# cropinghigh/sdrpp-dvbs-demodulator

Measured on AMD Instinct MI355X. Metric: Msymbols/s demod+FEC, DVB-S2 8PSK 3/4 normal-frame @50 LDPC iters, higher is better.
Workload: dtype int8 (FEC) / f32 (demod); 1 GPU; DVB-S2 8PSK 3/4 normal FECFRAME (MODCOD 14), pilots off, 27.5 Msym/s-class streams at 2 sps, carrier offset 1e-3 rad/sample, clock error ~10 ppm, Es/N0 11 dB, 50 forced LDPC iterations, IQ in -> BBFRAMEs out; streams_per_gpu=4096, symbols_per_frame=21690, distinct_signal_blocks=64, parallelism=independent transponder streams sharded over GPUs, no data-path collective, fec_pipelined_across_steps=True, ranks_seen_by_backend=1, backend=none

## Files before the change

### sdrpp-dvbs-demodulator_amd/csrc/ldpc_split_kernel.hip

```cpp
#include <hip/hip_runtime.h>
#include <stdint.h>
#include <algorithm>
#include "ldpc_lane_common.h"
#include "ldpc_split_plan.h"

namespace s2 {

#ifndef LDPC_SPLIT_EXP
#define LDPC_SPLIT_EXP 0
#endif
#ifndef LDPC_SPLIT_SKIP
#define LDPC_SPLIT_SKIP 0
#endif

template <int MAXDEG>
struct SplitShape {
    static constexpr int NL = MAXDEG + 2, HS = (NL + 1) / 2, NP = (HS + 1) / 2;
    static constexpr bool ODD = (NL & 1) != 0;
    static constexpr int PREV_SLOT = ODD ? HS - 2 : HS - 1;
    static constexpr int NPW = (HS / 2 + 1) <= 1 ? 1 : (HS / 2 + 1) <= 2 ? 2 : (HS / 2 + 1) <= 4 ? 4 : 8;
    static constexpr int REC = HS <= 4 ? 1 : HS <= 8 ? 2 : 4;
    static constexpr int RI_WORD = HS / 2, RI_SHIFT = (HS & 1) ? 16 : 0;
    static constexpr int NOPREV_SHARED = (MAXDEG == 4 || MAXDEG == 8) ? 2 : 0;
    static_assert(HS / 2 + 1 <= NPW, "slots + row word must fit the thread's table entry (ldpc_split_plan.h)");
// ... 103 lines not shown
        }
        if (S::ODD && ((HS - 1) >> 1) == p) {
            const bool me = (t & 1) != 0;
            constexpr int hh = (HS - 1) & 1;
            v[hh] = me ? (short)(127 << 8) : v[hh];
            g[hh] = me ? (short)(126 << 8) : g[hh];
        }
        R.V[p] = v; R.G[p] = g;
        if constexpr (LATE < 0) {
            if (p < -LATE) { v = late ? splat2(127 << 8) : v; g = late ? splat2(126 << 8) : g; }
        }
        if (p == 0) { MIN0 = g; }
        else if (p == 1) { MIN1 = pmax2(MIN0, g); MIN0 = pmin2(MIN0, g); }
        else { MIN1 = pmin2(MIN1, pmax2(MIN0, g)); MIN0 = pmin2(MIN0, g); }
        SX ^= bits2(v);
    }
    const int m0 = (int)bits2(pmin2(MIN0, swap2(MIN0)));
    const int m1 = (int)bits2(pmin2(pmax2(MIN0, swap2(MIN0)), pmin2(MIN1, swap2(MIN1))));
    const int sx = (int)(SX ^ __builtin_amdgcn_alignbit(SX, SX, 16));
    const int o0 = QUAD_DPP(m0, DPP_SWAP_HALVES), o1 = QUAD_DPP(m1, DPP_SWAP_HALVES), os = QUAD_DPP(sx, DPP_SWAP_HALVES);
    M1 = min(max(m0, o0), min(m1, o1));
    M0 = min(m0, o0);
    SXs = sx ^ os;
}

template <int MAXDEG, int LATE>
__device__ __forceinline__ void row_totals(const RowState<MAXDEG>& R, const uint32_t late, int& M0, int& M1, int& SXs) {
    using S = SplitShape<MAXDEG>;
    constexpr int NP = S::NP;
    s16x2 MIN0 = splat2(Q8_NONE), MIN1 = splat2(Q8_NONE);
    uint32_t SX = 0;
#pragma unroll
    for (int p = 0; p < NP; ++p) {
        s16x2 v = R.V[p], g = R.G[p];
        if constexpr (LATE < 0) {
            if (p < -LATE) { v = late ? splat2(127 << 8) : v; g = late ? splat2(126 << 8) : g; }
        }
        if (p == 0) { MIN0 = g; }
        else if (p == 1) { MIN1 = pmax2(MIN0, g); MIN0 = pmin2(MIN0, g); }
        else { MIN1 = pmin2(MIN1, pmax2(MIN0, g)); MIN0 = pmin2(MIN0, g); }
        SX ^= bits2(v);
    }
    const int m0 = (int)bits2(pmin2(MIN0, swap2(MIN0)));
    const int m1 = (int)bits2(pmin2(pmax2(MIN0, swap2(MIN0)), pmin2(MIN1, swap2(MIN1))));
    const int sx = (int)(SX ^ __builtin_amdgcn_alignbit(SX, SX, 16));
    const int o0 = QUAD_DPP(m0, DPP_SWAP_HALVES), o1 = QUAD_DPP(m1, DPP_SWAP_HALVES), os = QUAD_DPP(sx, DPP_SWAP_HALVES);
    M1 = min(max(m0, o0), min(m1, o1));
    M0 = min(m0, o0);
    SXs = sx ^ os;
}

template <int MAXDEG, int SKIP>
__device__ __forceinline__ void row_output(const RowState<MAXDEG>& R, const int M0, const int M1, const int SXs, const uint32_t early, uint32_t (&rec_out)[SplitShape<MAXDEG>::REC],
                                           uint32_t* pn0 = nullptr , const int npn = 1) {
    using S = SplitShape<MAXDEG>;
    constexpr int HS = S::HS, NP = S::NP, REC = S::REC;
    const uint32_t C32 = 0x20002000u;
    const uint32_t MIN1C = (uint32_t)min(M1, (int)C32);
    const uint32_t SUMC = (uint32_t)min(M0, (int)C32) + MIN1C;
    const uint32_t SXB = (uint32_t)SXs;
    s16x2 NM[NP + 1];
    NM[NP] = splat2(0);
#pragma unroll
    for (int p = 0; p < NP; ++p) {
        const s16x2 other = from_bits2(SUMC - bits2(pmin2(R.G[p], from_bits2(MIN1C))));
        const s16x2 neg = from_bits2(SXB ^ bits2(R.V[p])) >> 15;
        s16x2 nm = pmin2(from_bits2(bits2(other) ^ bits2(neg)) - neg, q8(31));
        const uint32_t pn = bits2(sat_add2(R.V[p], nm)) >> 8;
        if (p < npn && pn0) pn0[p] = pn;
#pragma unroll
        for (int hh = 0; hh < 2; ++hh) {
            const int k = 2 * p + hh;
            if (k >= HS) { nm[hh] = 0; continue; }
            if (k < SKIP) {
                if (!((early >> k) & 1)) { if (hh == 0) lds_write_lo_i8(R.addr[k], pn); else lds_write_hi_i8(R.addr[k], pn); }
            } else {
                if (hh == 0) lds_write_lo_i8(R.addr[k], pn); else lds_write_hi_i8(R.addr[k], pn);
            }
        }
        NM[p] = nm;
    }
#pragma unroll
    for (int w = 0; w < REC; ++w) {
        if (2 * w < NP) rec_out[w] = __builtin_amdgcn_perm(bits2(NM[2 * w + 1 <= NP ? 2 * w + 1 : NP]), bits2(NM[2 * w]), 0x07050301u);
        else rec_out[w] = 0;
    }
}

#if defined(LDPC_PROF) && LDPC_PROF == 3
#define SPLIT_MARK(i) do { if (KIND == 1 && g_prof_dev && blockIdx.x == 0 && (t == 0 || t == 384)) { const unsigned long long t_now = clock64(); g_prof_dev[300 + (t ? 16 : 0) + (i)] += t_now - t_mark; t_mark = t_now; } } while (0)
#define SPLIT_MARK_DECL unsigned long long t_mark = clock64()
__device__ unsigned long long* g_prof_dev = nullptr;
#else
#define SPLIT_MARK(i) do { } while (0)
#define SPLIT_MARK_DECL do { } while (0)
#endif
#define LINK_IN(k) ((int)R.V[(k) >> 1][(k) & 1] >> 8)
#define LINK_MG(k) ((int)R.G[(k) >> 1][(k) & 1] >> 8)
#define LINK_SET(k, v, m) do { R.V[(k) >> 1][(k) & 1] = (short)((v) << 8); R.G[(k) >> 1][(k) & 1] = (short)((m) << 8); } while (0)

__device__ __forceinline__ uint2 chain_record_x(const int m, const int qE, const int vE, const int sneg ) {
    const int sig = 1 | sneg;
    const int c31 = min(qE, 31), c32 = min(qE, 32);
    const int CA = (sneg ? c32 : c31) + 1, CB = (sneg ? c31 : c32) + 1;
    const uint32_t lim = ((uint32_t)(m + 1) & 0xffu) | (((uint32_t)(m + CA) & 0xffu) << 8) | (((uint32_t)(m - CB) & 0xffu) << 16) | ((uint32_t)(m - 1) << 24);
    const uint32_t se = ((uint32_t)(vE - 2 * sig * m - sneg) & 0xffffu) | (((uint32_t)sneg & 0xffu) << 16);
    return make_uint2(lim, se);
}
__device__ __forceinline__ int chain_step_x(const int x, const u32x2 r) {
    const int q1 = min(max(x, (int)(int8_t)r.x), (int)(int8_t)(r.x >> 8));
    const int q2 = min(max(x, (int)(int8_t)(r.x >> 16)), (int)r.x >> 24);
    int tx = (q1 + q2) ^ (int)(int8_t)(r.y >> 16);
    asm volatile("" : "+v"(tx));
    return clamp8(tx + (int)(short)r.y);
}
typedef __attribute__((address_space(3))) u32x2 lds_u2;
#define LDS_U2(a) (*(const lds_u2*)(uintptr_t)(a))
typedef u32x2 __attribute__((aligned(4))) u32x2_a4;
typedef __attribute__((address_space(3))) u32x2_a4 lds_u2_a4;
#define LDS_U2_A4(a) (*(const lds_u2_a4*)(uintptr_t)(a))

template <int MAXDEG>
__device__ __forceinline__ void chain_layer(RowState<MAXDEG>& R, uint32_t (&rec_out)[SplitShape<MAXDEG>::REC],
                                            const LdpcSplitLayer L, const uint32_t eL, const int t, int8_t* __restrict__ post, uint32_t* __restrict__ cw,
                                            const uint32_t flagb , const uint32_t cseq ,
                                            const bool fail_attempts ) {
    [[maybe_unused]] constexpr int KIND = 1;
    typedef __attribute__((address_space(3))) uint32_t lds_u1;
    const uint32_t rw = R.rw;
    const uint32_t level = rw & 0xffu, late = (rw >> 8) & 3u, early = (rw >> 12) & 3u;
    const int chain_d = (int)(L.aux & 0xffffu);
    const int j = t >> 1;
    const bool half1 = (t & 1) != 0;
    const uint32_t emask = ((early & 1u) ? 0xffu : 0u) | ((early & 2u) ? 0xff0000u : 0u);
    const uint32_t my_flag = flagb + 4u * (cseq & 1u);
    const bool attempt = (uint32_t)__builtin_amdgcn_readfirstlane((int)*(const lds_u1*)(uintptr_t)(flagb + 4u * ((cseq - 1u) & 1u))) != cseq - 1u;
    int M0, M1, SXs;
    uint32_t x0, pn0 = 0;
    SPLIT_MARK_DECL;
    row_input<MAXDEG, -1, SplitShape<MAXDEG>::NOPREV_SHARED>(R, (!attempt && level > 1u && !half1) ? 1u : 0u, 1u , t, M0, M1, SXs, ((L.kind_nw >> 20) & 1u) != 0, &x0);
    SPLIT_MARK(0);
    if (attempt) {
        row_output<MAXDEG, 2>(R, M0, M1, SXs, (level > 1u && !half1) ? 3u : 0u, rec_out, &pn0);
        const bool bad = fail_attempts || ((pn0 ^ (x0 >> 8)) & emask) != 0;
        if (__builtin_amdgcn_ballot_w64(bad) != 0 && (t & 63) == 0) *(lds_u1*)(uintptr_t)my_flag = cseq;
        lds_pairs_wait();
        lds_barrier();
        if ((uint32_t)__builtin_amdgcn_readfirstlane((int)*(const lds_u1*)(uintptr_t)my_flag) != cseq) {
            if (level > 1u && !half1) {
                if (!(early & 1u)) lds_write_lo_i8(R.addr[0], pn0);
                if (!(early & 2u)) lds_write_hi_i8(R.addr[1], pn0);
            }
            return;
        }
        row_totals<MAXDEG, -1>(R, (level > 1u && !half1) ? 1u : 0u, M0, M1, SXs);
    } else if (level == 1u) {
        row_output<MAXDEG, 0>(R, M0, M1, SXs, 0u, rec_out, &pn0);
    }
    if ((late >> 1) & 1) {
        reinterpret_cast<uint2*>(cw)[j] = chain_record_x(R.msg(1), (late & 1u) ? 255 : (M0 >> 24), (int)R.V[0][0] >> 8, SXs >> 31);
    }
    SPLIT_MARK(1);
    lds_pairs_wait();
    lds_barrier();
    SPLIT_MARK(2);
    uint32_t cwb = lds_offset(reinterpret_cast<const int8_t*>(cw));
    asm volatile("" : "+s"(cwb));
    if (t < chain_d) {
        __builtin_amdgcn_s_setprio(3);
        const int T = (int)(L.aux >> 16);
        int x = post[link_addr(eL, t + chain_d)];
        const uint32_t step = 8u * (uint32_t)chain_d, step4 = 4u * step;
        uint32_t p0 = cwb + 8u * (uint32_t)(t + chain_d), p1 = p0 + step, p2 = p1 + step, p3 = p2 + step;
        u32x2 r0 = LDS_U2(p0), r1 = LDS_U2(p1), r2 = LDS_U2(p2), r3 = LDS_U2(p3);
        int k = 1;
#define WALK_ROW(p, r) do { LDS_I8((p) + 7u) = (int8_t)x; x = chain_step_x(x, r); asm volatile("" : "+v"(p), "+v"(x) : : "memory"); } while (0)
        for (; k + 4 <= T; k += 4) {
            WALK_ROW(p0, r0); p0 += step4; r0 = LDS_U2(p0);
            WALK_ROW(p1, r1); p1 += step4; r1 = LDS_U2(p1);
            WALK_ROW(p2, r2); p2 += step4; r2 = LDS_U2(p2);
            WALK_ROW(p3, r3); p3 += step4; r3 = LDS_U2(p3);
        }
        if (k < T) {
            WALK_ROW(p0, r0); ++k;
            if (k < T) {
                WALK_ROW(p1, r1); ++k;
                if (k < T) { WALK_ROW(p2, r2); ++k; }
            }
        }
#undef WALK_ROW
        if (t + T * chain_d < 360) LDS_I8(cwb + 8u * (uint32_t)(t + T * chain_d) + 7u) = (int8_t)x;
        __builtin_amdgcn_s_setprio(0);
    }
    SPLIT_MARK(3);
    lds_barrier();
    SPLIT_MARK(4);
    if (level > 1u) {
        if (!half1) {
            uint32_t xr, xh;
            lds_read_pair_i8(R.addr[0], cwb + 8u * (uint32_t)j + 7u, xr, xh);
            lds_ready_n(0, xr, xh);
            const s16x2 X = from_bits2(__builtin_amdgcn_perm(xh, xr, 0x060c000cu));
            const s16x2 v = sat_sub2(X, R.RP[0]);
            const s16x2 av = pmax2(v, sat_sub2(splat2(0), v));
            const s16x2 g = __builtin_bit_cast(s16x2, __builtin_elementwise_sub_sat(__builtin_bit_cast(u16x2, av), (u16x2){256, 256}));
            const uint32_t rws = rw << 22;
            const uint32_t LM = __builtin_amdgcn_perm(rws << 1, rws, 0x09090b0bu);
            R.V[0] = from_bits2((bits2(v) & LM) | (bits2(R.V[0]) & ~LM));
            R.G[0] = from_bits2((bits2(g) & LM) | (bits2(R.G[0]) & ~LM));
            const int a = (int)bits2(pmin2(R.G[0], swap2(R.G[0]))), b = (int)bits2(pmax2(R.G[0], swap2(R.G[0])));
            M1 = min(M1, max(M0, a));
            M0 = min(M0, a);
            M1 = min(M1, max(M0, b));
            const uint32_t sv = bits2(R.V[0]);
            SXs ^= (int)(sv ^ __builtin_amdgcn_alignbit(sv, sv, 16));
        }
        M0 = QUAD_DPP(M0, DPP_FROM_HALF0);
        M1 = QUAD_DPP(M1, DPP_FROM_HALF0);
        SXs = QUAD_DPP(SXs, DPP_FROM_HALF0);
        SPLIT_MARK(5);
        row_output<MAXDEG, 2>(R, M0, M1, SXs, early, rec_out, &pn0);
    }
    if (!attempt) {
        const bool bad = ((pn0 ^ (x0 >> 8)) & emask) != 0;
        if (__builtin_amdgcn_ballot_w64(bad) != 0 && (t & 63) == 0) *(lds_u1*)(uintptr_t)my_flag = cseq;
    }
    SPLIT_MARK(6);
}

typedef const __attribute__((address_space(4))) uint32_t* const_u32_ptr;
typedef const __attribute__((address_space(4))) LdpcSplitLayer* const_layer_ptr;

__device__ __forceinline__ LdpcSplitLayer layer_at(const_layer_ptr layers, int i) {
    LdpcSplitLayer L;
    L.kind_nw = layers[i].kind_nw; L.aux = layers[i].aux; L.rec_off = layers[i].rec_off; L.ent_off = layers[i].ent_off;
    return L;
}
#ifndef LDPC_SPLIT_SPEC_STATS
#define LDPC_SPLIT_SPEC_STATS 0
#endif
template <int MAXDEG>
__device__ __forceinline__ void spec_layer(RowState<MAXDEG>& R, uint32_t (&rec_out)[SplitShape<MAXDEG>::REC], const LdpcSplitLayer L, const uint32_t* __restrict__ tab, const int t,
                                           uint32_t* __restrict__ cw, [[maybe_unused]] unsigned long long* prof, [[maybe_unused]] const int pl,
                                           const uint32_t vflagb , const uint32_t cseq ,
                                           const bool fail_attempts ) {
    static_assert(SplitShape<MAXDEG>::HS >= 4, "the shared links are slots 0..3 of half 0");
    typedef __attribute__((address_space(3))) uint32_t lds_u1;
    const uint32_t level = R.rw & 0xffu;
    const int j = t >> 1;
    const bool half1 = (t & 1) != 0;
    const bool spec = level > 1u && !half1;
    const int depth = (int)(L.aux >> 16);
    u32x2 side;
    {
        const uint64_t sbase = (uint64_t)(uintptr_t)(tab + L.ent_off);
        const uint32_t voff = (uint32_t)j * 8u;
        asm volatile("global_load_dwordx2 %0, %1, %2" : "=&v"(side) : "v"(voff), "s"(sbase) : "memory");
    }
    uint32_t cwb = lds_offset(reinterpret_cast<const int8_t*>(cw));
    asm volatile("" : "+s"(cwb));
    const uint32_t flagb = cwb + 4u * 384u;
    if (t == 0) { *(lds_u1*)(uintptr_t)flagb = 0u; *(lds_u1*)(uintptr_t)(flagb + 4u) = 0u; }
    const uint32_t my_flag = vflagb + 4u * (cseq & 1u);
    const bool attempt = (uint32_t)__builtin_amdgcn_readfirstlane((int)*(const lds_u1*)(uintptr_t)(vflagb + 4u * ((cseq - 1u) & 1u))) != cseq - 1u;
    u32x2 side_a = {0u, 0u};
    if (attempt) {
        const uint64_t sbase = (uint64_t)(uintptr_t)(tab + L.ent_off);
        const uint32_t voff = (uint32_t)j * 8u;
        asm volatile("global_load_dwordx2 %0, %1, %2" : "=&v"(side_a) : "v"(voff), "s"(sbase) : "memory");
    }
    int M0, M1, SXs;
    uint32_t xr[2], pn[2] = {0u, 0u};
    row_input<MAXDEG, -2, SplitShape<MAXDEG>::NOPREV_SHARED>(R, (!attempt && spec) ? 1u : 0u, 1u, t, M0, M1, SXs, ((L.kind_nw >> 20) & 1u) != 0, xr, 2);
    uint32_t em0 = 0, em1 = 0;
#if LDPC_SPLIT_SPEC_STATS
    if (prof && blockIdx.x == 0 && t == 0) { prof[900] += 1; prof[901] += attempt; prof[910 + (cseq < 40 ? cseq : 40)] += attempt; }
#endif
    if (attempt) {
        row_output<MAXDEG, 4>(R, M0, M1, SXs, spec ? 15u : 0u, rec_out, pn, 2);
        asm volatile("s_waitcnt vmcnt(0)" : "+v"(side_a) : : "memory");
        em0 = (((side_a.x >> 15) & 1u) ? 0xffu : 0u) | (((side_a.x >> 31) & 1u) ? 0xff0000u : 0u);
        em1 = (((side_a.y >> 15) & 1u) ? 0xffu : 0u) | (((side_a.y >> 31) & 1u) ? 0xff0000u : 0u);
        const bool bad = fail_attempts || (!half1 && ((((pn[0] ^ (xr[0] >> 8)) & em0) | ((pn[1] ^ (xr[1] >> 8)) & em1)) != 0));
        if (__builtin_amdgcn_ballot_w64(bad) != 0 && (t & 63) == 0) *(lds_u1*)(uintptr_t)my_flag = cseq;
        lds_pairs_wait();
        lds_barrier();
        if ((uint32_t)__builtin_amdgcn_readfirstlane((int)*(const lds_u1*)(uintptr_t)my_flag) != cseq) {
#if LDPC_SPLIT_SPEC_STATS
            if (prof && blockIdx.x == 0 && t == 0) prof[902] += 1;
#endif
            if (spec) {
                if (!(em0 & 0xffu)) lds_write_lo_i8(R.addr[0], pn[0]);
                if (!(em0 >> 16)) lds_write_hi_i8(R.addr[1], pn[0]);
                if (!(em1 & 0xffu)) lds_write_lo_i8(R.addr[2], pn[1]);
                if (!(em1 >> 16)) lds_write_hi_i8(R.addr[3], pn[1]);
            }
            return;
        }
        row_totals<MAXDEG, -2>(R, spec ? 1u : 0u, M0, M1, SXs);
    } else {
        if (level == 1u) row_output<MAXDEG, 0>(R, M0, M1, SXs, 0u, rec_out, pn, 2);
    }
    const uint32_t cell = cwb + 4u * (uint32_t)j;
    uint32_t cur[4];
#pragma unroll
    for (int s = 0; s < 4; ++s) cur[s] = R.addr[s];
    const s16x2 Q0 = from_bits2((uint32_t)min(M0 >> 24, 32) * 0x01000100u);
    const uint32_t s0w = (uint32_t)(SXs >> 31) & 0x80008000u;
    lds_pairs_wait();
    lds_barrier();
    s16x2 V0 = R.V[0], V1 = R.V[1];
    uint32_t X0p = 0, X1p = 0;
    int p = 0;
    bool voted = false;
    const bool any_spec = __builtin_amdgcn_ballot_w64(spec) != 0;
    for (;;) {
        bool ch = false;
        if (any_spec) {
            if (spec) {
                uint32_t xr0, xh0, xr1, xh1;
                lds_read_pair_i8(cur[0], cur[1], xr0, xh0);
                lds_read_pair_i8(cur[2], cur[3], xr1, xh1);
                lds_ready_n(0, xr0, xh0);
                asm volatile("" : "+v"(xr1), "+v"(xh1));
                const uint32_t X0 = __builtin_amdgcn_perm(xh0, xr0, 0x060c000cu), X1 = __builtin_amdgcn_perm(xh1, xr1, 0x060c000cu);
                ch = ((X0 ^ X0p) | (X1 ^ X1p)) != 0;
                X0p = X0; X1p = X1;
                V0 = sat_sub2(from_bits2(X0), R.RP[0]);
                V1 = sat_sub2(from_bits2(X1), R.RP[1]);
                const s16x2 G0 = __builtin_bit_cast(s16x2, __builtin_elementwise_sub_sat(__builtin_bit_cast(u16x2, pmax2(V0, sat_sub2(splat2(0), V0))), (u16x2){256, 256}));
                const s16x2 G1 = __builtin_bit_cast(s16x2, __builtin_elementwise_sub_sat(__builtin_bit_cast(u16x2, pmax2(V1, sat_sub2(splat2(0), V1))), (u16x2){256, 256}));
                const s16x2 P0 = pmin2(G0, swap2(G0)), P1 = pmin2(G1, swap2(G1));
                const s16x2 O0 = pmin2(pmin2(swap2(G0), P1), Q0), O1 = pmin2(pmin2(swap2(G1), P0), Q0);
                uint32_t sx = bits2(V0) ^ bits2(V1);
                sx ^= __builtin_amdgcn_alignbit(sx, sx, 16);
                sx ^= s0w;
                const s16x2 N0 = from_bits2(sx ^ bits2(V0)) >> 15, N1 = from_bits2(sx ^ bits2(V1)) >> 15;
                const s16x2 NM0 = pmin2(from_bits2(bits2(O0) ^ bits2(N0)) - N0, q8(31)), NM1 = pmin2(from_bits2(bits2(O1) ^ bits2(N1)) - N1, q8(31));
                *(lds_u1*)(uintptr_t)cell = __builtin_amdgcn_perm(bits2(sat_add2(V1, NM1)), bits2(sat_add2(V0, NM0)), 0x07050301u);
            }
        }
        if (p == 0) {
            asm volatile("s_waitcnt vmcnt(0)" : "+v"(side) : : "memory");
#pragma unroll
            for (int s = 0; s < 4; ++s) {
                const uint32_t f = ((s < 2 ? side.x : side.y) >> (16 * (s & 1))) & 0x7ffu;
                cur[s] = f ? cell - f : R.addr[s];
            }
        }
        ++p;
        if (p >= depth - 1) break;
        if (p > 1 && __builtin_amdgcn_ballot_w64(ch) != 0 && (t & 63) == 0) *(lds_u1*)(uintptr_t)(flagb + 4u * (uint32_t)(p & 1)) = (uint32_t)p + 1u;
        lds_pairs_wait();
        lds_barrier();
        if (p > 1) {
            const uint32_t fl = (uint32_t)__builtin_amdgcn_readfirstlane((int)*(const lds_u1*)(uintptr_t)(flagb + 4u * (uint32_t)(p & 1)));
            if (fl != (uint32_t)p + 1u) { voted = true; break; }
        }
    }
#if LDPC_SPLIT_SPEC_STATS
    if (prof && blockIdx.x == 0 && t == 0) prof[512 + 32 * (pl % 11) + (p < 31 ? p : 31)] += 1;
#endif
    if (!voted) { lds_pairs_wait(); lds_barrier(); }
    if (level > 1u) {
        if (!half1) {
            R.V[0] = V0; R.V[1] = V1;
#pragma unroll
            for (int q = 0; q < 2; ++q) {
                R.G[q] = __builtin_bit_cast(s16x2, __builtin_elementwise_sub_sat(__builtin_bit_cast(u16x2, pmax2(R.V[q], sat_sub2(splat2(0), R.V[q]))), (u16x2){256, 256}));
                const int a = (int)bits2(pmin2(R.G[q], swap2(R.G[q]))), b = (int)bits2(pmax2(R.G[q], swap2(R.G[q])));
                M1 = min(M1, max(M0, a));
                M0 = min(M0, a);
                M1 = min(M1, max(M0, b));
            }
            const uint32_t sv = bits2(R.V[0]) ^ bits2(R.V[1]);
            SXs ^= (int)(sv ^ __builtin_amdgcn_alignbit(sv, sv, 16));
        }
        M0 = QUAD_DPP(M0, DPP_FROM_HALF0);
        M1 = QUAD_DPP(M1, DPP_FROM_HALF0);
        SXs = QUAD_DPP(SXs, DPP_FROM_HALF0);
        const uint32_t early = ((side.x >> 15) & 1u) | ((side.x >> 30) & 2u) | ((side.y >> 13) & 4u) | ((side.y >> 28) & 8u);
        row_output<MAXDEG, 4>(R, M0, M1, SXs, half1 ? 0u : early, rec_out, pn, 2);
    }
    if (!attempt) {
        em0 = (((side.x >> 15) & 1u) ? 0xffu : 0u) | (((side.x >> 31) & 1u) ? 0xff0000u : 0u);
        em1 = (((side.y >> 15) & 1u) ? 0xffu : 0u) | (((side.y >> 31) & 1u) ? 0xff0000u : 0u);
        const bool bad = !half1 && ((((pn[0] ^ (xr[0] >> 8)) & em0) | ((pn[1] ^ (xr[1] >> 8)) & em1)) != 0);
        if (__builtin_amdgcn_ballot_w64(bad) != 0 && (t & 63) == 0) *(lds_u1*)(uintptr_t)my_flag = cseq;
    }
}
#undef LINK_IN
#undef LINK_MG
#undef LINK_SET

template <int MAXDEG>
__global__ __launch_bounds__(LDPC_SPLIT_T) __attribute__((amdgpu_waves_per_eu(8))) void ldpc_split_kernel(LdpcKernelParams read_through_ldpc_params) {
    using S = SplitShape<MAXDEG>;
    constexpr int T = LDPC_SPLIT_T, REC = S::REC, NPW = S::NPW;
    extern __shared__ __attribute__((aligned(16))) int8_t lds_all[];
    const int t = threadIdx.x;
    const int wave = __builtin_amdgcn_readfirstlane(t >> 6);
    int8_t* __restrict__ post = lds_all;

#if defined(LDPC_PROF) && LDPC_PROF == 3
    if (blockIdx.x == 0) g_prof_dev = ldpc_params()->A.prof;
    __syncthreads();
#endif
    int f = blockIdx.x;
    while (f < ldpc_params()->A.nframes) {
        {
            const LdpcKernelParamsPtr P = ldpc_params();
            const int N = P->A.N, K = P->A.K, R = P->A.R, q = P->A.q;
            uint32_t* __restrict__ msg = P->A.msg_ws + (size_t)blockIdx.x * (size_t)P->A.pent_base;
            const int8_t* __restrict__ src = P->A.llr + (size_t)f * N;
            int t = threadIdx.x;
            asm volatile("" : "+v"(t));
            ldpc_frame_load<T>(post, src, K, R, q, t);
            for (uint32_t o = (uint32_t)t; o < (uint32_t)P->A.pent_base; o += T) msg[o] = 0;
            if (t < 2) reinterpret_cast<uint32_t*>(lds_all + ((N + LDPC_SPLIT_SCRATCH + 15) & ~15) + 8 * 360)[t] = 0;
        }
        __syncthreads();

        int it = 0, ret = 0;
        uint32_t cseq = 0;
        while (true) {
            const LdpcKernelParamsPtr P = ldpc_params();
            const LdpcKernelArgs A = ldpc_args(P);
            const int N = A.N, q = A.q, npl = P->npl;
            const const_layer_ptr layers = (const_layer_ptr)P->layers;
            const const_u32_ptr ents = (const_u32_ptr)P->ents;
            const int npad = (N + LDPC_SPLIT_SCRATCH + 15) & ~15;
            uint32_t* __restrict__ cw = reinterpret_cast<uint32_t*>(lds_all + npad);
            int* __restrict__ s_flag = reinterpret_cast<int*>(lds_all + N);
            const uint32_t cflagb = (uint32_t)npad + 8u * 360u;
            uint32_t* __restrict__ msg = A.msg_ws + (size_t)blockIdx.x * (size_t)A.pent_base;
            uint32_t* __restrict__ sgn = A.sgn_ws + (size_t)blockIdx.x * SGN_WS_DWORDS;
            const __amdgpu_buffer_rsrc_t rs_tab = wave_entries_rsrc<NPW>(const_cast<uint32_t*>(P->atab), wave, P->tab_words);
            const __amdgpu_buffer_rsrc_t rs_msg = wave_entries_rsrc<REC>(msg, wave, A.pent_base);
            const bool check = !A.force || it == A.max_trials;
            if (check) {
// ... 1 lines not shown
                const unsigned long long tc0 = clock64();
#endif
                const uint32_t zflag = sign_pack(post, N, reinterpret_cast<uint8_t*>(sgn), t, T);
#if defined(LDPC_PROF) && LDPC_PROF == 5
                const unsigned long long tc1 = clock64();
#endif
                __syncthreads();
#if defined(LDPC_PROF) && LDPC_PROF == 5
                const unsigned long long tc2 = clock64();
#endif
                const bool bad = zflag != 0 || syndromes_bad<MAXDEG>(q, A.synd_base, P->ents, sgn, t, T);
                const unsigned long long b = __ballot(bad);
#if defined(LDPC_PROF) && LDPC_PROF == 5
                const unsigned long long tc3 = clock64();
#endif
                if ((t & 63) == 0) s_flag[t >> 6] = (b != 0);
                lds_barrier();
                int any = 0;
#pragma unroll
                for (int w = 0; w < T / 64; ++w) any |= s_flag[w];
                any = __builtin_amdgcn_readfirstlane(any);
                lds_barrier();
#if defined(LDPC_PROF) && LDPC_PROF == 5
                if (A.prof && blockIdx.x == 0 && t == 0) { const unsigned long long tc4 = clock64(); A.prof[400] += tc1 - tc0; A.prof[401] += tc2 - tc1; A.prof[402] += tc3 - tc2; A.prof[403] += tc4 - tc3; A.prof[404] += 1; }
#endif
                if (A.force) { ret = any ? -1 : A.max_trials; break; }
                if (!any) { ret = it; break; }
                if (it == A.max_trials) { ret = -1; break; }
            }
            typename FetchWords<REC>::type rec_n;
            typename FetchWords<NPW>::type pw_n;
            LdpcSplitLayer Lnext = layer_at(layers, 0), Lnext2 = layer_at(layers, npl > 1 ? 1 : 0);
            uint32_t soff_tab = 0;
            pw_n = bload<NPW>(rs_tab, soff_tab);
            rec_n = bload<REC>(rs_msg, Lnext.rec_off * 4u);
            asm volatile("" : "+v"(rec_n), "+v"(pw_n));
#if defined(LDPC_PROF)
            unsigned long long t_layer = clock64();
            if (A.prof && blockIdx.x == 0 && t == 0) { A.prof[127] += t_layer - A.prof[126]; }
#endif
            for (int pl = 0; pl < npl; ++pl) {
                const LdpcSplitLayer L = Lnext;
                Lnext = Lnext2;
                Lnext2 = layer_at(layers, pl + 2 < npl ? pl + 2 : npl - 1);
                soff_tab += T * NPW * 4;
                RowState<MAXDEG> RS;
                RS.unpack(pw_n, rec_n);
                RS.pin();
                asm volatile("" : "+v"(pw_n), "+v"(rec_n));
                if (pl + 1 < npl && !(LDPC_SPLIT_EXP & 2)) {
                    if (!(LDPC_SPLIT_EXP & 16)) pw_n = bload<NPW>(rs_tab, soff_tab);
                    if (!(LDPC_SPLIT_EXP & 32)) rec_n = bload<REC>(rs_msg, Lnext.rec_off * 4u);
                }
                auto thread_index = [&]() __attribute__((always_inline)) { int tt = t; asm volatile("" : "+v"(tt)); return tt; };
                const uint32_t kind = L.kind_nw & 0xffu;
                uint32_t ro[REC];
                if (LDPC_SPLIT_SKIP && ((LDPC_SPLIT_SKIP >> kind) & 1)) {
#pragma unroll
                    for (int w = 0; w < REC; ++w) ro[w] = RS.rw;
                } else if (kind == 0) {
                    int M0, M1, SXs;
                    row_input<MAXDEG, 0>(RS, 0u, 0u, S::ODD ? thread_index() : t, M0, M1, SXs);
                    if (LDPC_SPLIT_EXP & 8) { ro[0] = (uint32_t)(M0 ^ M1 ^ SXs); ro[REC - 1] = ro[0]; }
                    else row_output<MAXDEG, 0>(RS, M0, M1, SXs, 0u, ro);
                } else if (kind == 7) {
                    int M0, M1, SXs;
                    row_input<MAXDEG, 0, 1>(RS, 0u, L.aux, thread_index(), M0, M1, SXs);
                    row_output<MAXDEG, 0>(RS, M0, M1, SXs, 0u, ro);
                } else if (kind == 1) {
                    ++cseq;
                    chain_layer<MAXDEG>(RS, ro, L, ents[L.ent_off + 1], thread_index(), post, cw, cflagb, cseq, A.dbg != 0);
                } else {
                    ++cseq;
                    if constexpr (S::HS >= 4) spec_layer<MAXDEG>(RS, ro, L, P->atab, thread_index(), cw, A.prof, pl, cflagb, cseq, A.dbg != 0);
                }
#if defined(LDPC_PROF) && LDPC_PROF == 4
                const unsigned long long t_claim = clock64();
#endif
                asm volatile("" : "+v"(rec_n), "+v"(pw_n));
#if defined(LDPC_PROF) && LDPC_PROF == 4
                if (A.prof && blockIdx.x == 0 && (t == 0 || t == 384)) A.prof[200 + pl + (t ? 50 : 0)] += clock64() - t_claim;
#endif
                if (LDPC_SPLIT_EXP & (2 | 64)) asm volatile("" :: "v"(ro[0]), "v"(ro[REC - 1]));
                else bstore<REC>(ro, rs_msg, L.rec_off * 4u);
                lds_pairs_wait();
                if (!(LDPC_SPLIT_EXP & 4)) lds_barrier();
#if defined(LDPC_PROF)
                if (A.prof && blockIdx.x == 0 && t == 0) { const unsigned long long t_now = clock64(); A.prof[128 + pl] += t_now - t_layer; t_layer = t_now; A.prof[126] = t_now; }
#endif
            }
            ++it;
        }

        {
            const LdpcKernelParamsPtr P = ldpc_params();
            const LdpcKernelArgs A = ldpc_args(P);
            const int N = A.N, K = A.K, R = A.R, q = A.q;
            int* __restrict__ s_flag = reinterpret_cast<int*>(lds_all + N);
            int t = threadIdx.x;
            asm volatile("" : "+v"(t));
            ldpc_frame_store<T>(post, f, ret, A.trials, A.hard, A.hard_stride, A.post, N, K, R, q, t, wave);
            if (A.work_ctr) {
                if (t == 0) s_flag[12] = (int)(gridDim.x + atomicAdd(A.work_ctr, 1u));
                lds_barrier();
                f = __builtin_amdgcn_readfirstlane(s_flag[12]);
            } else {
                f += gridDim.x;
            }
        }
        __syncthreads();
    }
}

size_t ldpc_split_lds_bytes(int N) {
    const size_t npad = (size_t)((N + LDPC_SPLIT_SCRATCH + 15) & ~15);
    return npad + 8 * 360 + 16;
}
size_t ldpc_split_msg_bytes_per_block(const LdpcDeviceCode& C) { return (size_t)C.split_rec_total * sizeof(uint32_t); }

template <int MAXDEG>
static hipError_t launch_split(const LdpcDeviceCode& C, const LdpcKernelArgs& A, int grid, hipStream_t stream) {
    LdpcKernelParams P;
    P.A = A; P.layers = C.d_split_layers; P.ents = C.d_ents; P.atab = C.d_split_atab; P.rows = C.d_rows; P.npl = C.split_npl; P.tab_words = C.split_tab_words;
    return ldpc_launch(ldpc_split_kernel<MAXDEG>, grid, LDPC_SPLIT_T, ldpc_split_lds_bytes(A.N), stream, P);
}
template <int MAXDEG>
static int occupancy_split(int N) { return ldpc_occupancy(ldpc_split_kernel<MAXDEG>, LDPC_SPLIT_T, ldpc_split_lds_bytes(N)); }
// ... 31 lines not shown
```

### sdrpp-dvbs-demodulator_amd/csrc/ldpc_split_plan.h

```cpp
#pragma once
#include "ldpc_plan.h"

namespace s2 {

constexpr int LDPC_SPLIT_T = 768;
constexpr int LDPC_SPLIT_SCRATCH = 64;
#ifndef LDPC_SPLIT_SPEC_MIN_T
#define LDPC_SPLIT_SPEC_MIN_T 64
#endif

struct LdpcSplitLayer {
    uint32_t kind_nw;
    uint32_t aux;
    uint32_t rec_off;
    uint32_t ent_off;
};

struct LdpcSplitPlan {
    bool ok = false;
    const char* why = "";
    int hs = 0;
    int npw = 0;
    int rec_dwords = 0;
    int rec_total = 0;
    int chain_layers = 0;
    bool noprev_shared = false;
    std::vector<LdpcSplitLayer> layers;
    std::vector<uint32_t> atab;
    std::vector<uint32_t> side;
    std::vector<int> row_of;
    std::vector<int> layer_of;
};

inline int ldpc_split_npw(int hs) {
    const int words = hs / 2 + 1;
    return words <= 1 ? 1 : words <= 2 ? 2 : words <= 4 ? 4 : 8;
}

inline int ldpc_split_plan_rec_dwords(int max_deg) { const int hs = (max_deg + 3) / 2; return hs <= 4 ? 1 : hs <= 8 ? 2 : 4; }

inline LdpcSplitPlan build_ldpc_split_plan(const LdpcPlan& P) {
    LdpcSplitPlan S;
    const int NL = P.max_deg + 2;
    if (P.min_deg != P.max_deg || (NL + 1) / 2 > 14 || P.N + LDPC_SPLIT_SCRATCH > 65536) { S.why = "irregular row degree, more than 14 slots per half or more than 65 472 bits"; return S; }
    for (const LdpcLayerDesc& L : P.layers) {
        const int nc = (int)(L.depth_nc >> 16), depth = (int)(L.depth_nc & 0xffffu);
        if (depth > 1 && (nc > 4 || nc > (NL + 1) / 2)) { S.why = "a layer with more than four shared links"; return S; }
    }
    S.hs = (NL + 1) / 2;
    S.npw = ldpc_split_npw(S.hs);
    S.rec_dwords = ldpc_split_plan_rec_dwords(P.max_deg);
    const int q = P.q, K = P.K, N = P.N, T = LDPC_SPLIT_T, hs = S.hs, npw = S.npw;
    auto scratch = [&](int t) { return (uint32_t)(N + (t & (LDPC_SPLIT_SCRATCH - 1))); };
    auto slot_addr = [&](int i, int j, int k) -> uint32_t {
        const LdpcLayerDesc& L = P.layers[i];
        if (k < P.max_deg) {
            const uint32_t e = P.ents[L.ent_off + k];
            return 360u * (e >> 16) + ((uint32_t)j + (e & 0xffffu)) % 360u;
        }
        if (k == P.max_deg) return (uint32_t)(K + 360 * i + j);
        if (i > 0) return (uint32_t)(K + 360 * (i - 1) + j);
        if (j > 0) return (uint32_t)(K + 360 * (q - 1) + j - 1);
        return ~0u;
    };
    std::vector<std::pair<int, std::vector<uint32_t>>> side_of;
    bool bad_noprev = false;
    auto emit = [&](int kind, int i, const std::vector<int>& rows, const std::vector<uint32_t>* info, uint32_t aux) {
        LdpcSplitLayer D{};
        const int nw = T / 64;
        D.kind_nw = (uint32_t)kind | ((uint32_t)nw << 8) | ((kind != 0 ? (P.layers[i].depth_nc >> 16) : 0u) << 16);
        D.aux = aux;
        D.rec_off = (uint32_t)S.rec_total;
        D.ent_off = P.layers[i].ent_off;
        S.rec_total += nw * 64 * S.rec_dwords;
        const size_t base = S.atab.size();
        S.atab.resize(base + (size_t)T * npw, 0);
        const size_t rbase = S.row_of.size();
        S.row_of.resize(rbase + T / 2, -1);
        for (int t = 0; t < T; ++t) {
            uint32_t* w = &S.atab[base + (size_t)t * npw];
            const int pr = t >> 1, h = t & 1;
            const int j = pr < (int)rows.size() ? rows[pr] : -1;
            for (int s = 0; s < hs; ++s) {
                uint32_t a = scratch(t);
                if (j >= 0 && h * hs + s < NL) {
                    a = slot_addr(i, j, h * hs + s);
                    if (a == ~0u) { a = scratch(t); D.kind_nw |= 1u << 20; if (kind == 0) { D.aux = (uint32_t)t; D.kind_nw = (D.kind_nw & ~0xffu) | 7u; } else bad_noprev = true; }
                }
                w[s >> 1] |= a << (16 * (s & 1));
            }
            if (j >= 0 && h == 0) S.row_of[rbase + pr] = j;
            if (j >= 0 && info && (h == 0 || kind == 1 || kind == 8)) w[hs >> 1] |= ((*info)[pr] & (h == 1 ? 0xffu : 0xffffu)) << (16 * (hs & 1));
        }
        S.layers.push_back(D);
        S.layer_of.push_back(i);
    };
    for (int i = 0; i < q; ++i) {
        const LdpcLayerDesc& L = P.layers[i];
        const int depth = (int)(L.depth_nc & 0xffffu);
        const uint32_t chain = L.deg >> 16;
        std::vector<int> rows;
        if (depth == 1) {
            for (int j = 0; j < 360; ++j) rows.push_back(j);
            emit(0, i, rows, nullptr, 0);
        } else {
            std::vector<uint32_t> info;
            for (int j = 0; j < 360; ++j) {
                const uint32_t rw = P.rows[L.row_off + j];
                rows.push_back(j);
                info.push_back((rw & 0xffu) | (((rw >> 8) & 15u) << 8) | (((rw >> 20) & 15u) << 12));
            }
            if (chain != 0 && chain != LDPC_WALK_MARK && 359u / chain < (uint32_t)LDPC_SPLIT_SPEC_MIN_T) emit(1, i, rows, &info, chain | ((359u / chain) << 16));
            else {
                std::map<uint32_t, std::pair<int, int>> last;
                std::vector<int> lvl(360, 1);
                std::vector<uint32_t> side(2 * 384, 0);
                int depth8 = 1;
                for (int j = 0; j < 360; ++j) {
                    std::pair<int, int> pred[4] = {{-1, 0}, {-1, 0}, {-1, 0}, {-1, 0}};
                    for (int k = 0; k < NL; ++k) {
                        const uint32_t a = slot_addr(i, j, k);
                        if (a == ~0u) continue;
                        auto it = last.find(a);
                        if (it != last.end()) {
                            if (k >= 4 || k >= hs) { LdpcSplitPlan F; F.why = "a shared link outside slots 0..3 of half 0"; return F; }
                            pred[k] = it->second;
                            lvl[j] = std::max(lvl[j], lvl[it->second.first] + 1);
                            side[2 * it->second.first + (it->second.second >> 1)] |= 0x8000u << (16 * (it->second.second & 1));
                        }
                        last[a] = {j, k};
                    }
                    depth8 = std::max(depth8, lvl[j]);
                    for (int k = 0; k < 4; ++k)
                        if (pred[k].first >= 0 && lvl[pred[k].first] > 1) side[2 * j + (k >> 1)] |= (uint32_t)(4 * (j - pred[k].first) - pred[k].second) << (16 * (k & 1));
                }
                if (depth8 > 255 || hs < 4) { LdpcSplitPlan F; F.why = "a speculative layer deeper than 255 levels or fewer than 4 slots per half"; return F; }
                for (int j = 0; j < 360; ++j) info[j] = (uint32_t)lvl[j];
                emit(8, i, rows, &info, (uint32_t)depth8 << 16);
                side_of.push_back({(int)S.layers.size() - 1, side});
            }
            S.chain_layers++;
        }
    }
    for (auto& so : side_of) {
        S.layers[so.first].ent_off = (uint32_t)(S.atab.size() + S.side.size());
        S.side.insert(S.side.end(), so.second.begin(), so.second.end());
    }
    S.ok = true;
    S.noprev_shared = bad_noprev;
    return S;
}

}
```

Before: 2802 Msymbols/s.

## Precompute per-row hold/early flags in plan and streamline speculative attempt path

Result: no change. 2831 Msymbols/s, median of 6 (+1.1%).

```diff
diff --git a/sdrpp-dvbs-demodulator_amd/csrc/ldpc_split_kernel.hip b/sdrpp-dvbs-demodulator_amd/csrc/ldpc_split_kernel.hip
--- a/sdrpp-dvbs-demodulator_amd/csrc/ldpc_split_kernel.hip
+++ b/sdrpp-dvbs-demodulator_amd/csrc/ldpc_split_kernel.hip
@@ -179,7 +179,9 @@
 
 template <int MAXDEG, int SKIP>
 __device__ __forceinline__ void row_output(const RowState<MAXDEG>& R, const int M0, const int M1, const int SXs, const uint32_t early, uint32_t (&rec_out)[SplitShape<MAXDEG>::REC],
-                                           uint32_t* pn0 = nullptr , const int npn = 1) {
+                                           uint32_t* pn0 = nullptr , const int npn = 1,
+                                           uint32_t* dq0 = nullptr ,
+                                           const bool hold = false ) {
     using S = SplitShape<MAXDEG>;
     constexpr int HS = S::HS, NP = S::NP, REC = S::REC;
     const uint32_t C32 = 0x20002000u;
@@ -193,14 +195,16 @@
         const s16x2 other = from_bits2(SUMC - bits2(pmin2(R.G[p], from_bits2(MIN1C))));
         const s16x2 neg = from_bits2(SXB ^ bits2(R.V[p])) >> 15;
         s16x2 nm = pmin2(from_bits2(bits2(other) ^ bits2(neg)) - neg, q8(31));
-        const uint32_t pn = bits2(sat_add2(R.V[p], nm)) >> 8;
+        const uint32_t pq = bits2(sat_add2(R.V[p], nm));
+        const uint32_t pn = pq >> 8;
         if (p < npn && pn0) pn0[p] = pn;
+        if (p < npn && dq0) dq0[p] ^= pq;
 #pragma unroll
         for (int hh = 0; hh < 2; ++hh) {
             const int k = 2 * p + hh;
             if (k >= HS) { nm[hh] = 0; continue; }
             if (k < SKIP) {
-                if (!((early >> k) & 1)) { if (hh == 0) lds_write_lo_i8(R.addr[k], pn); else lds_write_hi_i8(R.addr[k], pn); }
+                if (!(hold || ((early >> (15 - k)) & 1))) { if (hh == 0) lds_write_lo_i8(R.addr[k], pn); else lds_write_hi_i8(R.addr[k], pn); }
             } else {
                 if (hh == 0) lds_write_lo_i8(R.addr[k], pn); else lds_write_hi_i8(R.addr[k], pn);
             }
@@ -217,8 +221,10 @@
 #if defined(LDPC_PROF) && LDPC_PROF == 3
 #define SPLIT_MARK(i) do { if (KIND == 1 && g_prof_dev && blockIdx.x == 0 && (t == 0 || t == 384)) { const unsigned long long t_now = clock64(); g_prof_dev[300 + (t ? 16 : 0) + (i)] += t_now - t_mark; t_mark = t_now; } } while (0)
 #define SPLIT_MARK_DECL unsigned long long t_mark = clock64()
+#define SPLIT_MARK_READS_T 1
 __device__ unsigned long long* g_prof_dev = nullptr;
 #else
+#define SPLIT_MARK_READS_T 0
 #define SPLIT_MARK(i) do { } while (0)
 #define SPLIT_MARK_DECL do { } while (0)
 #endif
@@ -247,43 +253,75 @@
 typedef __attribute__((address_space(3))) u32x2_a4 lds_u2_a4;
 #define LDS_U2_A4(a) (*(const lds_u2_a4*)(uintptr_t)(a))
 
-template <int MAXDEG>
+template <int NS>
+__device__ __forceinline__ void early_masks_q8(const uint32_t rw, uint32_t (&em)[NS / 2]) {
+    if constexpr (NS == 2) {
+        em[0] = __builtin_amdgcn_perm(rw << 1, rw, 0x0a0c080cu);
+    } else {
+        const uint32_t z = rw | (rw << 18), z1 = z << 1;
+        em[0] = __builtin_amdgcn_perm(z1, z, 0x0a0c080cu);
+        em[1] = __builtin_amdgcn_perm(z1, z, 0x0b0c090cu);
+    }
+}
+
+template <int MAXDEG, int NS>
+__device__ __forceinline__ bool attempt_layer(RowState<MAXDEG>& R, uint32_t (&rec_out)[SplitShape<MAXDEG>::REC], const int t, const bool noprev_rt,
+                                              const uint32_t my_flag , const uint32_t cseq, const bool fail_attempts) {
+    typedef __attribute__((address_space(3))) uint32_t lds_u1;
+    constexpr int NPS = NS / 2;
+    asm volatile("" : "+v"(R.rw));
+    const uint32_t rw = R.rw;
+    int M0, M1, SXs;
+    uint32_t dq[NPS], pn[NPS], em[NPS];
+    row_input<MAXDEG, 0, SplitShape<MAXDEG>::NOPREV_SHARED>(R, 0u, 1u , t, M0, M1, SXs, noprev_rt, dq, NPS);
+    const bool hold = (rw & LDPC_SPLIT_RW_HOLD) != 0;
+    row_output<MAXDEG, NS>(R, M0, M1, SXs, 0u, rec_out, pn, NPS, dq, hold);
+    early_masks_q8<NS>(rw, em);
+    uint32_t changed = dq[0] & em[0];
+    if constexpr (NPS == 2) changed |= dq[1] & em[1];
+    if (__builtin_expect(__builtin_amdgcn_ballot_w64(changed != 0) != 0 || fail_attempts, 0)) *(lds_u1*)(uintptr_t)my_flag = cseq;
+    lds_pairs_wait();
+    lds_barrier();
+    if ((uint32_t)__builtin_amdgcn_readfirstlane((int)*(const lds_u1*)(uintptr_t)my_flag) == cseq) return false;
+    auto held = [&](int k) { return (rw & (LDPC_SPLIT_RW_HOLD | (LDPC_SPLIT_RW_EARLY0 >> k))) == LDPC_SPLIT_RW_HOLD; };
+    if (held(0)) lds_write_lo_i8(R.addr[0], pn[0]);
+    if (held(1)) lds_write_hi_i8(R.addr[1], pn[0]);
+    if constexpr (NPS == 2) {
+        if (held(2)) lds_write_lo_i8(R.addr[2], pn[1]);
+        if (held(3)) lds_write_hi_i8(R.addr[3], pn[1]);
+    }
+    return true;
+}
+
+template <int MAXDEG, class ThreadIndex>
 __device__ __forceinline__ void chain_layer(RowState<MAXDEG>& R, uint32_t (&rec_out)[SplitShape<MAXDEG>::REC],
-                                            const LdpcSplitLayer L, const uint32_t eL, const int t, int8_t* __restrict__ post, uint32_t* __restrict__ cw,
+                                            const LdpcSplitLayer L, const uint32_t eL, const ThreadIndex& thread_index, int8_t* __restrict__ post, uint32_t* __restrict__ cw,
                                             const uint32_t flagb , const uint32_t cseq ,
                                             const bool fail_attempts ) {
     [[maybe_unused]] constexpr int KIND = 1;
     typedef __attribute__((address_space(3))) uint32_t lds_u1;
-    const uint32_t rw = R.rw;
-    const uint32_t level = rw & 0xffu, late = (rw >> 8) & 3u, early = (rw >> 12) & 3u;
     const int chain_d = (int)(L.aux & 0xffffu);
-    const int j = t >> 1;
-    const bool half1 = (t & 1) != 0;
-    const uint32_t emask = ((early & 1u) ? 0xffu : 0u) | ((early & 2u) ? 0xff0000u : 0u);
     const uint32_t my_flag = flagb + 4u * (cseq & 1u);
     const bool attempt = (uint32_t)__builtin_amdgcn_readfirstlane((int)*(const lds_u1*)(uintptr_t)(flagb + 4u * ((cseq - 1u) & 1u))) != cseq - 1u;
     int M0, M1, SXs;
-    uint32_t x0, pn0 = 0;
+    uint32_t x0 = 0;
     SPLIT_MARK_DECL;
-    row_input<MAXDEG, -1, SplitShape<MAXDEG>::NOPREV_SHARED>(R, (!attempt && level > 1u && !half1) ? 1u : 0u, 1u , t, M0, M1, SXs, ((L.kind_nw >> 20) & 1u) != 0, &x0);
-    SPLIT_MARK(0);
+    constexpr bool T_IN_ATTEMPT = SplitShape<MAXDEG>::ODD || SplitShape<MAXDEG>::NOPREV_SHARED != 0 || SPLIT_MARK_READS_T != 0;
+    int t = 0;
+    if constexpr (T_IN_ATTEMPT) t = thread_index();
     if (attempt) {
-        row_output<MAXDEG, 2>(R, M0, M1, SXs, (level > 1u && !half1) ? 3u : 0u, rec_out, &pn0);
-        const bool bad = fail_attempts || ((pn0 ^ (x0 >> 8)) & emask) != 0;
-        if (__builtin_amdgcn_ballot_w64(bad) != 0 && (t & 63) == 0) *(lds_u1*)(uintptr_t)my_flag = cseq;
-        lds_pairs_wait();
-        lds_barrier();
-        if ((uint32_t)__builtin_amdgcn_readfirstlane((int)*(const lds_u1*)(uintptr_t)my_flag) != cseq) {
-            if (level > 1u && !half1) {
-                if (!(early & 1u)) lds_write_lo_i8(R.addr[0], pn0);
-                if (!(early & 2u)) lds_write_hi_i8(R.addr[1], pn0);
-            }
-            return;
-        }
-        row_totals<MAXDEG, -1>(R, (level > 1u && !half1) ? 1u : 0u, M0, M1, SXs);
-    } else if (level == 1u) {
-        row_output<MAXDEG, 0>(R, M0, M1, SXs, 0u, rec_out, &pn0);
-    }
+        if (attempt_layer<MAXDEG, 2>(R, rec_out, t, ((L.kind_nw >> 20) & 1u) != 0, my_flag, cseq, fail_attempts)) return;
+        row_totals<MAXDEG, -1>(R, (R.rw & LDPC_SPLIT_RW_HOLD) ? 1u : 0u, M0, M1, SXs);
+    } else {
+        row_input<MAXDEG, -1, SplitShape<MAXDEG>::NOPREV_SHARED>(R, (R.rw & LDPC_SPLIT_RW_HOLD) ? 1u : 0u, 1u , t, M0, M1, SXs, ((L.kind_nw >> 20) & 1u) != 0, &x0);
+        SPLIT_MARK(0);
+        if ((R.rw & 0xffu) == 1u) row_output<MAXDEG, 0>(R, M0, M1, SXs, 0u, rec_out, nullptr, 1, &x0);
+    }
+    if constexpr (!T_IN_ATTEMPT) t = thread_index();
+    const uint32_t rw = R.rw;
+    const uint32_t level = rw & 0xffu, late = (rw >> LDPC_SPLIT_RW_LATE_SHIFT) & 3u;
+    const bool hold = (rw & LDPC_SPLIT_RW_HOLD) != 0;
+    const int j = t >> 1;
     if ((late >> 1) & 1) {
         reinterpret_cast<uint2*>(cw)[j] = chain_record_x(R.msg(1), (late & 1u) ? 255 : (M0 >> 24), (int)R.V[0][0] >> 8, SXs >> 31);
     }
@@ -323,7 +361,7 @@
     lds_barrier();
     SPLIT_MARK(4);
     if (level > 1u) {
-        if (!half1) {
+        if (hold) {
             uint32_t xr, xh;
             lds_read_pair_i8(R.addr[0], cwb + 8u * (uint32_t)j + 7u, xr, xh);
             lds_ready_n(0, xr, xh);
@@ -331,7 +369,7 @@
             const s16x2 v = sat_sub2(X, R.RP[0]);
             const s16x2 av = pmax2(v, sat_sub2(splat2(0), v));
             const s16x2 g = __builtin_bit_cast(s16x2, __builtin_elementwise_sub_sat(__builtin_bit_cast(u16x2, av), (u16x2){256, 256}));
-            const uint32_t rws = rw << 22;
+            const uint32_t rws = rw << (30 - LDPC_SPLIT_RW_LATE_SHIFT);
             const uint32_t LM = __builtin_amdgcn_perm(rws << 1, rws, 0x09090b0bu);
             R.V[0] = from_bits2((bits2(v) & LM) | (bits2(R.V[0]) & ~LM));
             R.G[0] = from_bits2((bits2(g) & LM) | (bits2(R.G[0]) & ~LM));
@@ -346,10 +384,12 @@
         M1 = QUAD_DPP(M1, DPP_FROM_HALF0);
         SXs = QUAD_DPP(SXs, DPP_FROM_HALF0);
         SPLIT_MARK(5);
-        row_output<MAXDEG, 2>(R, M0, M1, SXs, early, rec_out, &pn0);
+        row_output<MAXDEG, 2>(R, M0, M1, SXs, rw, rec_out, nullptr, 1, &x0);
     }
     if (!attempt) {
-        const bool bad = ((pn0 ^ (x0 >> 8)) & emask) != 0;
+        uint32_t em[1];
+        early_masks_q8<2>(rw, em);
+        const bool bad = (x0 & em[0]) != 0;
         if (__builtin_amdgcn_ballot_w64(bad) != 0 && (t & 63) == 0) *(lds_u1*)(uintptr_t)my_flag = cseq;
     }
     SPLIT_MARK(6);
@@ -366,68 +406,51 @@
 #ifndef LDPC_SPLIT_SPEC_STATS
 #define LDPC_SPLIT_SPEC_STATS 0
 #endif
-template <int MAXDEG>
-__device__ __forceinline__ void spec_layer(RowState<MAXDEG>& R, uint32_t (&rec_out)[SplitShape<MAXDEG>::REC], const LdpcSplitLayer L, const uint32_t* __restrict__ tab, const int t,
+template <int MAXDEG, class ThreadIndex>
+__device__ __forceinline__ void spec_layer(RowState<MAXDEG>& R, uint32_t (&rec_out)[SplitShape<MAXDEG>::REC], const LdpcSplitLayer L, const uint32_t* __restrict__ tab, const ThreadIndex& thread_index,
                                            uint32_t* __restrict__ cw, [[maybe_unused]] unsigned long long* prof, [[maybe_unused]] const int pl,
                                            const uint32_t vflagb , const uint32_t cseq ,
                                            const bool fail_attempts ) {
     static_assert(SplitShape<MAXDEG>::HS >= 4, "the shared links are slots 0..3 of half 0");
     typedef __attribute__((address_space(3))) uint32_t lds_u1;
-    const uint32_t level = R.rw & 0xffu;
-    const int j = t >> 1;
-    const bool half1 = (t & 1) != 0;
-    const bool spec = level > 1u && !half1;
     const int depth = (int)(L.aux >> 16);
     u32x2 side;
+    uint32_t cwb = lds_offset(reinterpret_cast<const int8_t*>(cw));
+    asm volatile("" : "+s"(cwb));
+    const uint32_t flagb = cwb + 4u * 384u;
+    const uint32_t my_flag = vflagb + 4u * (cseq & 1u);
+    const bool attempt = (uint32_t)__builtin_amdgcn_readfirstlane((int)*(const lds_u1*)(uintptr_t)(vflagb + 4u * ((cseq - 1u) & 1u))) != cseq - 1u;
+    int M0, M1, SXs;
+    uint32_t xr[2] = {0u, 0u};
+    constexpr bool T_IN_ATTEMPT = SplitShape<MAXDEG>::ODD || SplitShape<MAXDEG>::NOPREV_SHARED != 0 || LDPC_SPLIT_SPEC_STATS != 0;
+    int t = 0;
+    if constexpr (T_IN_ATTEMPT) t = thread_index();
+#if LDPC_SPLIT_SPEC_STATS
+    if (prof && blockIdx.x == 0 && t == 0) { prof[900] += 1; prof[901] += attempt; prof[910 + (cseq < 40 ? cseq : 40)] += attempt; }
+#endif
+    if (attempt) {
+        if (attempt_layer<MAXDEG, 4>(R, rec_out, t, ((L.kind_nw >> 20) & 1u) != 0, my_flag, cseq, fail_attempts)) {
+#if LDPC_SPLIT_SPEC_STATS
+            if (prof && blockIdx.x == 0 && t == 0) prof[902] += 1;
+#endif
+            return;
+        }
+        row_totals<MAXDEG, -2>(R, (R.rw & LDPC_SPLIT_RW_HOLD) ? 1u : 0u, M0, M1, SXs);
+    } else {
+        row_input<MAXDEG, -2, SplitShape<MAXDEG>::NOPREV_SHARED>(R, (R.rw & LDPC_SPLIT_RW_HOLD) ? 1u : 0u, 1u, t, M0, M1, SXs, ((L.kind_nw >> 20) & 1u) != 0, xr, 2);
+        if ((R.rw & 0xffu) == 1u) row_output<MAXDEG, 0>(R, M0, M1, SXs, 0u, rec_out, nullptr, 2, xr);
+    }
+    if constexpr (!T_IN_ATTEMPT) t = thread_index();
+    const uint32_t rw = R.rw;
+    const uint32_t level = rw & 0xffu;
+    const int j = t >> 1;
+    const bool spec = (rw & LDPC_SPLIT_RW_HOLD) != 0;
     {
         const uint64_t sbase = (uint64_t)(uintptr_t)(tab + L.ent_off);
         const uint32_t voff = (uint32_t)j * 8u;
         asm volatile("global_load_dwordx2 %0, %1, %2" : "=&v"(side) : "v"(voff), "s"(sbase) : "memory");
     }
-    uint32_t cwb = lds_offset(reinterpret_cast<const int8_t*>(cw));
-    asm volatile("" : "+s"(cwb));
-    const uint32_t flagb = cwb + 4u * 384u;
     if (t == 0) { *(lds_u1*)(uintptr_t)flagb = 0u; *(lds_u1*)(uintptr_t)(flagb + 4u) = 0u; }
-    const uint32_t my_flag = vflagb + 4u * (cseq & 1u);
-    const bool attempt = (uint32_t)__builtin_amdgcn_readfirstlane((int)*(const lds_u1*)(uintptr_t)(vflagb + 4u * ((cseq - 1u) & 1u))) != cseq - 1u;
-    u32x2 side_a = {0u, 0u};
-    if (attempt) {
-        const uint64_t sbase = (uint64_t)(uintptr_t)(tab + L.ent_off);
-        const uint32_t voff = (uint32_t)j * 8u;
-        asm volatile("global_load_dwordx2 %0, %1, %2" : "=&v"(side_a) : "v"(voff), "s"(sbase) : "memory");
-    }
-    int M0, M1, SXs;
-    uint32_t xr[2], pn[2] = {0u, 0u};
-    row_input<MAXDEG, -2, SplitShape<MAXDEG>::NOPREV_SHARED>(R, (!attempt && spec) ? 1u : 0u, 1u, t, M0, M1, SXs, ((L.kind_nw >> 20) & 1u) != 0, xr, 2);
-    uint32_t em0 = 0, em1 = 0;
-#if LDPC_SPLIT_SPEC_STATS
-    if (prof && blockIdx.x == 0 && t == 0) { prof[900] += 1; prof[901] += attempt; prof[910 + (cseq < 40 ? cseq : 40)] += attempt; }
-#endif
-    if (attempt) {
-        row_output<MAXDEG, 4>(R, M0, M1, SXs, spec ? 15u : 0u, rec_out, pn, 2);
-        asm volatile("s_waitcnt vmcnt(0)" : "+v"(side_a) : : "memory");
-        em0 = (((side_a.x >> 15) & 1u) ? 0xffu : 0u) | (((side_a.x >> 31) & 1u) ? 0xff0000u : 0u);
-        em1 = (((side_a.y >> 15) & 1u) ? 0xffu : 0u) | (((side_a.y >> 31) & 1u) ? 0xff0000u : 0u);
-        const bool bad = fail_attempts || (!half1 && ((((pn[0] ^ (xr[0] >> 8)) & em0) | ((pn[1] ^ (xr[1] >> 8)) & em1)) != 0));
-        if (__builtin_amdgcn_ballot_w64(bad) != 0 && (t & 63) == 0) *(lds_u1*)(uintptr_t)my_flag = cseq;
-        lds_pairs_wait();
-        lds_barrier();
-        if ((uint32_t)__builtin_amdgcn_readfirstlane((int)*(const lds_u1*)(uintptr_t)my_flag) != cseq) {
-#if LDPC_SPLIT_SPEC_STATS
-            if (prof && blockIdx.x == 0 && t == 0) prof[902] += 1;
-#endif
-            if (spec) {
-                if (!(em0 & 0xffu)) lds_write_lo_i8(R.addr[0], pn[0]);
-                if (!(em0 >> 16)) lds_write_hi_i8(R.addr[1], pn[0]);
-                if (!(em1 & 0xffu)) lds_write_lo_i8(R.addr[2], pn[1]);
-                if (!(em1 >> 16)) lds_write_hi_i8(R.addr[3], pn[1]);
-            }
-            return;
-        }
-        row_totals<MAXDEG, -2>(R, spec ? 1u : 0u, M0, M1, SXs);
-    } else {
-        if (level == 1u) row_output<MAXDEG, 0>(R, M0, M1, SXs, 0u, rec_out, pn, 2);
-    }
     const uint32_t cell = cwb + 4u * (uint32_t)j;
     uint32_t cur[4];
 #pragma unroll
@@ -490,7 +513,7 @@
 #endif
     if (!voted) { lds_pairs_wait(); lds_barrier(); }
     if (level > 1u) {
-        if (!half1) {
+        if (spec) {
             R.V[0] = V0; R.V[1] = V1;
 #pragma unroll
             for (int q = 0; q < 2; ++q) {
@@ -506,13 +529,12 @@
         M0 = QUAD_DPP(M0, DPP_FROM_HALF0);
         M1 = QUAD_DPP(M1, DPP_FROM_HALF0);
         SXs = QUAD_DPP(SXs, DPP_FROM_HALF0);
-        const uint32_t early = ((side.x >> 15) & 1u) | ((side.x >> 30) & 2u) | ((side.y >> 13) & 4u) | ((side.y >> 28) & 8u);
-        row_output<MAXDEG, 4>(R, M0, M1, SXs, half1 ? 0u : early, rec_out, pn, 2);
+        row_output<MAXDEG, 4>(R, M0, M1, SXs, rw, rec_out, nullptr, 2, xr);
     }
     if (!attempt) {
-        em0 = (((side.x >> 15) & 1u) ? 0xffu : 0u) | (((side.x >> 31) & 1u) ? 0xff0000u : 0u);
-        em1 = (((side.y >> 15) & 1u) ? 0xffu : 0u) | (((side.y >> 31) & 1u) ? 0xff0000u : 0u);
-        const bool bad = !half1 && ((((pn[0] ^ (xr[0] >> 8)) & em0) | ((pn[1] ^ (xr[1] >> 8)) & em1)) != 0);
+        uint32_t em[2];
+        early_masks_q8<4>(rw, em);
+        const bool bad = ((xr[0] & em[0]) | (xr[1] & em[1])) != 0;
         if (__builtin_amdgcn_ballot_w64(bad) != 0 && (t & 63) == 0) *(lds_u1*)(uintptr_t)my_flag = cseq;
     }
 }
@@ -620,7 +642,12 @@
                     if (!(LDPC_SPLIT_EXP & 16)) pw_n = bload<NPW>(rs_tab, soff_tab);
                     if (!(LDPC_SPLIT_EXP & 32)) rec_n = bload<REC>(rs_msg, Lnext.rec_off * 4u);
                 }
-                auto thread_index = [&]() __attribute__((always_inline)) { int tt = t; asm volatile("" : "+v"(tt)); return tt; };
+                auto thread_index = [&]() __attribute__((always_inline)) {
+                    if constexpr (S::ODD) { int tt = t; asm volatile("" : "+v"(tt)); return tt; }
+                    uint32_t first = (uint32_t)wave << 6;
+                    asm volatile("" : "+s"(first));
+                    return (int)__builtin_amdgcn_mbcnt_hi(~0u, __builtin_amdgcn_mbcnt_lo(~0u, first));
+                };
                 const uint32_t kind = L.kind_nw & 0xffu;
                 uint32_t ro[REC];
                 if (LDPC_SPLIT_SKIP && ((LDPC_SPLIT_SKIP >> kind) & 1)) {
@@ -637,10 +664,10 @@
                     row_output<MAXDEG, 0>(RS, M0, M1, SXs, 0u, ro);
                 } else if (kind == 1) {
                     ++cseq;
-                    chain_layer<MAXDEG>(RS, ro, L, ents[L.ent_off + 1], thread_index(), post, cw, cflagb, cseq, A.dbg != 0);
+                    chain_layer<MAXDEG>(RS, ro, L, ents[L.ent_off + 1], thread_index, post, cw, cflagb, cseq, A.dbg != 0);
                 } else {
                     ++cseq;
-                    if constexpr (S::HS >= 4) spec_layer<MAXDEG>(RS, ro, L, P->atab, thread_index(), cw, A.prof, pl, cflagb, cseq, A.dbg != 0);
+                    if constexpr (S::HS >= 4) spec_layer<MAXDEG>(RS, ro, L, P->atab, thread_index, cw, A.prof, pl, cflagb, cseq, A.dbg != 0);
                 }
 #if defined(LDPC_PROF) && LDPC_PROF == 4
                 const unsigned long long t_claim = clock64();
diff --git a/sdrpp-dvbs-demodulator_amd/csrc/ldpc_split_plan.h b/sdrpp-dvbs-demodulator_amd/csrc/ldpc_split_plan.h
--- a/sdrpp-dvbs-demodulator_amd/csrc/ldpc_split_plan.h
+++ b/sdrpp-dvbs-demodulator_amd/csrc/ldpc_split_plan.h
@@ -31,6 +31,14 @@
     std::vector<int> row_of;
     std::vector<int> layer_of;
 };
+
+constexpr uint32_t LDPC_SPLIT_RW_LATE_SHIFT = 9, LDPC_SPLIT_RW_HOLD = 1u << 11, LDPC_SPLIT_RW_EARLY0 = 1u << 15;
+inline uint32_t ldpc_split_row_word(int half, uint32_t level, uint32_t late , uint32_t early ) {
+    uint32_t w = level & 0xffu;
+    if (half != 0) return w;
+    for (int k = 0; k < 4; ++k) w |= ((early >> k) & 1u) ? LDPC_SPLIT_RW_EARLY0 >> k : 0u;
+    return w | ((late & 3u) << LDPC_SPLIT_RW_LATE_SHIFT) | (level > 1u ? LDPC_SPLIT_RW_HOLD : 0u);
+}
 
 inline int ldpc_split_npw(int hs) {
     const int words = hs / 2 + 1;
@@ -90,7 +98,7 @@
                 w[s >> 1] |= a << (16 * (s & 1));
             }
             if (j >= 0 && h == 0) S.row_of[rbase + pr] = j;
-            if (j >= 0 && info && (h == 0 || kind == 1 || kind == 8)) w[hs >> 1] |= ((*info)[pr] & (h == 1 ? 0xffu : 0xffffu)) << (16 * (hs & 1));
+            if (j >= 0 && info) { const uint32_t rw = (*info)[pr]; w[hs >> 1] |= ldpc_split_row_word(h, rw & 0xffu, (rw >> 8) & 3u, (rw >> 12) & 15u) << (16 * (hs & 1)); }
         }
         S.layers.push_back(D);
         S.layer_of.push_back(i);
@@ -135,7 +143,11 @@
                         if (pred[k].first >= 0 && lvl[pred[k].first] > 1) side[2 * j + (k >> 1)] |= (uint32_t)(4 * (j - pred[k].first) - pred[k].second) << (16 * (k & 1));
                 }
                 if (depth8 > 255 || hs < 4) { LdpcSplitPlan F; F.why = "a speculative layer deeper than 255 levels or fewer than 4 slots per half"; return F; }
-                for (int j = 0; j < 360; ++j) info[j] = (uint32_t)lvl[j];
+                for (int j = 0; j < 360; ++j) {
+                    uint32_t early = 0;
+                    for (int k = 0; k < 4; ++k) early |= ((side[2 * j + (k >> 1)] >> (16 * (k & 1) + 15)) & 1u) << k;
+                    info[j] = (uint32_t)lvl[j] | (early << 12);
+                }
                 emit(8, i, rows, &info, (uint32_t)depth8 << 16);
                 side_of.push_back({(int)S.layers.size() - 1, side});
             }
```
